# finlaymiller/torch-vae

Hardware: AMD Instinct MI355X
Metric: training samples/sec (VAE step: forward+ELBO+backward+AdamW), synthetic pianoroll (higher is better)
Workload: dtype bf16; 1 GPU; VanillaVAE latent_dim=16, 128x128 synthetic pianoroll, batch 256/GPU (generalised bottleneck 256*(H/16)^2); img_size=128, latent_dim=16, batch_per_gpu=256, global_batch=256, parallelism=dp1, optimizer=AdamW+OneCycle (encoder, decoder groups)

## Files before the change

### torch_vae_amd/csrc/vae_api.hip

```cpp
#include <map>
#include <mutex>
#include "vae_ctx.h"
#include "edge_kernels.cuh"
#include "loglik.cuh"
#include "latent_stats.cuh"
#include "grad_clip.cuh"
#include "total_corr.cuh"

static thread_local std::string g_err;
int vae_set_error(const char* what, const char* why) {
    g_err = std::string(what) + ": " + why;
    return -1;
}

extern "C" const char* vae_last_error(void) { return g_err.c_str(); }
extern "C" int vae_abi_version(void) { return 1; }

static void param_shapes(int H, int L, int gen, int64_t* sizes) {
    const int s = gen ? H / 16 : 2;
    const int64_t F = 256LL * s * s;
    const int enc_ci[4] = {1, 32, 64, 128}, enc_co[4] = {32, 64, 128, 256};
    int k = 0;
    for (int i = 0; i < 4; ++i) { sizes[k++] = 9LL * enc_ci[i] * enc_co[i]; sizes[k++] = enc_co[i]; sizes[k++] = enc_co[i]; sizes[k++] = enc_co[i]; }
    sizes[k++] = L * F; sizes[k++] = L; sizes[k++] = L * F; sizes[k++] = L; sizes[k++] = F * L; sizes[k++] = F;
    const int dec_ci[3] = {256, 128, 64}, dec_co[3] = {128, 64, 32};
    for (int i = 0; i < 3; ++i) { sizes[k++] = 9LL * dec_ci[i] * dec_co[i]; sizes[k++] = dec_co[i]; sizes[k++] = dec_co[i]; sizes[k++] = dec_co[i]; }
    sizes[k++] = 9 * 32 * 32; sizes[k++] = 32; sizes[k++] = 32; sizes[k++] = 32; sizes[k++] = 9 * 32; sizes[k++] = 1;
}

extern "C" int vae_param_layout(int H, int L, int gen, int64_t* offsets, int64_t* sizes, int64_t* total) {
    if (H < 32 || (H & (H - 1)) || (!gen && H != 32)) return vae_set_error("vae_param_layout", "img_size must be a power of two >= 32 (exactly 32 unless generalised)");
    if (L < 1 || L > 4096) return vae_set_error("vae_param_layout", "latent_dim must be in 1..4096");
    param_shapes(H, L, gen, sizes);
    int64_t off = 0;
    for (int i = 0; i < VAE_NUM_PARAMS; ++i) { offsets[i] = off; off += align_up(sizes[i], 64); }
    *total = off;
    return 0;
}
extern "C" int vae_bn_layout(int64_t* offsets, int64_t* channels, int64_t* total) {
    int64_t off = 0;
    for (int i = 0; i < 8; ++i) { offsets[i] = off; channels[i] = kBnC[i]; off += 2 * kBnC[i]; }
    *total = off;
    return 0;
}

template <typename T> static T* dalloc(vae_ctx* c, size_t n) {
    void* p = nullptr;
    if (hipMalloc(&p, std::max<size_t>(n * sizeof(T), 256)) != hipSuccess) return nullptr;
    c->allocs.push_back(p); c->ws_bytes += (int64_t)std::max<size_t>(n * sizeof(T), 256);
    return reinterpret_cast<T*>(p);
}

struct DevStreams { hipStream_t side[vae_ctx::NSIDE]; hipStream_t comm; };
static DevStreams* device_streams(int side_prio) {
    static std::mutex mu;
    static std::map<int, DevStreams*> pool;
    int dev = 0;
    if (hipGetDevice(&dev) != hipSuccess) return nullptr;
    std::lock_guard<std::mutex> lk(mu);
    auto it = pool.find(dev);
    if (it != pool.end()) return it->second;
    DevStreams* d = new DevStreams();
    bool ok = true;
    for (int i = 0; i < vae_ctx::NSIDE && ok; ++i) ok = hipStreamCreateWithPriority(&d->side[i], hipStreamNonBlocking, side_prio) == hipSuccess;
    {
        int lo = 0, hi = 0;
        (void)hipDeviceGetStreamPriorityRange(&lo, &hi);
        const char* e = getenv("VAE_COMM_STREAM_PRIO");
        if (e && (!strcmp(e, "high") || !strcmp(e, "low"))) ok = ok && hipStreamCreateWithPriority(&d->comm, hipStreamNonBlocking, !strcmp(e, "high") ? hi : lo) == hipSuccess;
        else ok = ok && hipStreamCreateWithFlags(&d->comm, hipStreamNonBlocking) == hipSuccess;
    }
    if (!ok) { delete d; return nullptr; }
    pool[dev] = d;
    return d;
}

extern "C" void vae_destroy(vae_ctx* c) {
    if (!c) return;
    (void)vae_comm_destroy(c);
    for (void* p : c->allocs) (void)hipFree(p);
    if (c->ll_kb) (void)hipFree(c->ll_kb);
    if (c->n_side_ok) {
        for (int i = 0; i < vae_ctx::NSIDE; ++i) { (void)hipStreamSynchronize(c->side[i]); (void)hipEventDestroy(c->ev_join[i]); }
        (void)hipStreamSynchronize(c->comm);
        for (int i = 0; i < vae_ctx::NFORK; ++i) (void)hipEventDestroy(c->ev_fork[i]);
        (void)hipEventDestroy(c->ev_pack); (void)hipEventDestroy(c->ev_comm);
        if (c->ev_kl) (void)hipEventDestroy(c->ev_kl);
        for (int i = 0; i < vae_ctx::NBUCKET; ++i) (void)hipEventDestroy(c->ev_bucket[i]);
    }
    delete c;
}
extern "C" int64_t vae_workspace_bytes(const vae_ctx* c) { return c ? c->ws_bytes : 0; }

struct OptionDef { const char* name; int& (*ref)(vae_ctx&); int def; int (*norm)(int); };
static int opt_any(int v) { return v; }
static int opt_min1(int v) { return std::max(1, v); }
static int opt_fused_grid(int v) { return std::max(1, std::min(v, 512)); }
static int opt_max1024(int v) { return std::min(v, 1024); }
static int opt_max48(int v) { return std::min(v, 48); }
static int opt_fused_wgrad(int v) { return v == 1 ? 3 : v == 2 ? 1 : v == 3 ? 2 : 0; }
#define OPT(member, def, norm) {#member, [](vae_ctx& c) -> int& { return c.member; }, def, norm}
#define OPT_WK(member, def, norm) {"knob_wgrad_" #member, [](vae_ctx& c) -> int& { return c.wk.member; }, def, norm}
static const OptionDef kOptions[] = {
    OPT(use_tr16, 1, opt_any), OPT(use_mfma_convout, 1, opt_any), OPT(use_pipelined, 1, opt_any), OPT(use_side_stream, 1, opt_any),
    OPT(use_fused_bn, 1, opt_any), OPT(use_fused_convout, 1, opt_any), OPT(use_fused_wgrad, 1, opt_fused_wgrad), OPT(use_recomp_dz, 0, opt_any),
    OPT(use_raw_wgrad, 0, opt_any), OPT(use_deep, 1, opt_any), OPT(use_latent_mfma, 6, opt_any), OPT(use_convout_stream, 1, opt_any),
    OPT(use_dnf_stream, 1, opt_any), OPT(use_upf_stream, 1, opt_any), OPT(use_fc_dgrad8, 1, opt_any), OPT(use_wgrad_split, 1, opt_any),
    OPT(knob_up_per_cu, 2, opt_any), OPT(knob_down_per_cu, 2, opt_min1), OPT(knob_bwd_per_cu, 0, opt_any), OPT(knob_nt_max, 4, opt_any),
    OPT(knob_up_nt_max, 1, opt_min1), OPT(knob_wave_nt_max, 4, opt_any), OPT(knob_lay22_min_nt, 2, opt_any), OPT(knob_lay42, 1, opt_any),
    OPT(knob_down_waves, 8, opt_any), OPT(knob_pipe_max_cout, 256, opt_any), OPT(knob_xcd_map, 1, opt_any), OPT(knob_rev, 4, opt_any),
    OPT(knob_lean, 1, opt_any), OPT(knob_pack_grid, 128, opt_min1), OPT(knob_conv1_grid, 512, opt_any), OPT(knob_fused_grid, 256, opt_fused_grid),
    OPT(knob_convout_grid, 1536, opt_any), OPT(knob_convout_bwd_grid, 1024, opt_any), OPT(knob_convout_step_grid, 1024, opt_min1),
    OPT(knob_convout_bands, 0, opt_any), OPT(knob_wgrad_layer_wgs, 0, opt_any), OPT(knob_skip_wgrad, 0, opt_any), OPT(knob_ablate_b, 0, opt_any),
    OPT(knob_ablate_f, 0, opt_any),
    OPT_WK(tile, 1, opt_any), OPT_WK(wide, 1, opt_any), OPT_WK(mid8, 0, opt_any), OPT_WK(force_simple, 0, opt_any),
    OPT_WK(wgs, 128, opt_max1024), OPT_WK(wide_wgs, 128, opt_max1024), OPT_WK(cap_mb, 48, opt_max48),
};
#undef OPT_WK
#undef OPT
static const OptionDef* find_option(const char* name) {
    for (const OptionDef& o : kOptions) if (name && !strcmp(name, o.name)) return &o;
    return nullptr;
}

extern "C" vae_ctx* vae_create(int H, int L, int maxB, int dtype, int gen) {
    vae_ctx* c = new vae_ctx();
    c->H = H; c->L = L; c->maxB = maxB; c->dtype = dtype; c->gen = gen;
    for (const OptionDef& o : kOptions) o.ref(*c) = o.norm(o.def);
    if (getenv("VAE_NO_SIDE_STREAM")) c->use_side_stream = 0;
    if (vae_param_layout(H, L, gen, c->poff, c->psz, &c->ptotal) != 0) { delete c; return nullptr; }
    if (dtype != VAE_DTYPE_F32 && dtype != VAE_DTYPE_BF16 && dtype != VAE_DTYPE_F16) { vae_set_error("vae_create", "bad dtype"); delete c; return nullptr; }
    if (maxB < 1) { vae_set_error("vae_create", "max_batch < 1"); delete c; return nullptr; }
    vae_bn_layout(c->bnoff, c->bnc, &c->bntotal);
    c->s = gen ? H / 16 : 2; c->s2 = c->s * c->s; c->F = 256LL * c->s2;
    c->npad_fc = (int)align_up(2 * L, 32); c->npad_di = (int)align_up(L, 32);
    c->esz = dtype == VAE_DTYPE_F32 ? 4 : 2;
    const size_t B = maxB;
    const int hs[8] = {H / 2, H / 4, H / 8, H / 16, 2 * c->s, 4 * c->s, 8 * c->s, 16 * c->s};
    size_t nd = 0;
    for (int i = 0; i < 8; ++i) nd += 4 * kBnC[i];
    nd *= STAT_R;
    c->n_dstats = nd + 8 * STAT_R;
    c->dstats = dalloc<double>(c, c->n_dstats);
    bool ok = c->dstats != nullptr;
    double* dp = c->dstats;
    for (int i = 0; i < 8 && ok; ++i) {
        BnLayer& l = c->lay[i];
        l.C = kBnC[i]; l.H = hs[i]; l.W = hs[i];
        l.stat_f = dp; dp += 2 * l.C * STAT_R;
        const size_t n = B * l.H * l.W * l.C;
        l.y = dalloc<char>(c, n * c->esz); l.dz = dalloc<char>(c, n * c->esz); l.block = dalloc<float>(c, LC_ROWS * l.C);
        ok = l.y && l.dz && l.block;
        const int base = i < 4 ? 4 * i : (i < 7 ? 22 + 4 * (i - 4) : 34);
        l.p_convw = base; l.p_convb = base + 1; l.p_gamma = base + 2; l.p_beta = base + 3;
    }
    for (int i = 0; i < 8; ++i) { c->lay[i].stat_b = dp; dp += 2 * kBnC[i] * STAT_R; }
    c->accum = dp;
    if (ok) {
        c->d0 = dalloc<char>(c, B * c->F * c->esz); c->dd0 = dalloc<char>(c, B * c->F * c->esz);
        c->eps = dalloc<float>(c, B * L); c->dlat = dalloc<float>(c, B * 2 * L);
        c->dlogit = dalloc<float>(c, B * H * H); c->dlogit2 = dalloc<float>(c, B * H * H); c->ident = dalloc<float>(c, 3 * 256); c->wout_t = dalloc<float>(c, 288);
        ok = c->d0 && c->dd0 && c->eps && c->dlat && c->dlogit && c->dlogit2 && c->ident && c->wout_t;
    }
    const int ci[8] = {1, 32, 64, 128, 256, 128, 64, 32}, co[8] = {32, 64, 128, 256, 128, 64, 32, 32};
    for (int i = 1; i < 8 && ok; ++i) {
        const size_t n = (size_t)9 * ci[i] * co[i];
        c->wp_fwd[i] = dalloc<char>(c, n * c->esz); c->wp_dg[i] = dalloc<char>(c, n * c->esz);
        ok = c->wp_fwd[i] && c->wp_dg[i];
    }
    if (ok) {
        c->fcpack = dalloc<char>(c, (size_t)c->F * c->npad_fc * c->esz);
        c->dipack = dalloc<char>(c, (size_t)c->F * c->npad_di * c->esz);
        c->d_descs = dalloc<PackDesc>(c, 32);
        ok = c->fcpack && c->dipack && c->d_descs;
    }
    size_t slab = 2048 * 288;
    if (ok) {
        int a, b2, wa, wb;
        for (int wide = 0; wide < 2; ++wide)
            for (int big = 0; big < 2; ++big) {
                if (wide && dtype == VAE_DTYPE_F32) continue;
                for (int i = 1; i < 4; ++i) slab = std::max(slab, wgrad_slab_floats(c->wk, maxB, c->lay[i].H, c->lay[i].W, co[i], ci[i], &a, &b2, &wa, &wb, wide != 0, big != 0));
                for (int i = 4; i < 8; ++i) slab = std::max(slab, wgrad_slab_floats(c->wk, maxB, c->lay[i].H / 2, c->lay[i].W / 2, ci[i], co[i], &a, &b2, &wa, &wb, wide != 0, big != 0));
            }
        const size_t ksteps = c->F / 16;
        slab = std::max(slab, (size_t)std::min<size_t>(ksteps, 512) * maxB * c->npad_fc);
        slab = std::max(slab, (size_t)std::min<size_t>(ksteps, 512) * maxB * c->npad_di);
        slab = std::max(slab, (size_t)8 * (2 * (size_t)L * c->F + c->F));
        c->slab_floats = slab;
        c->slab = dalloc<float>(c, slab);
// ... 933 lines not shown
```

### torch_vae_amd/csrc/vae_ctx.h

```cpp
#pragma once
#include <hip/hip_runtime.h>
#include <stdio.h>
#include <string.h>
#include <math.h>
#include <string>
#include <vector>
#include <algorithm>

#include "../../include/vae_step.h"

int vae_set_error(const char* what, const char* why);

#include "common.cuh"

#define LAUNCH_CHECK(name)                                                        \
    do {                                                                          \
        hipError_t _e = hipGetLastError();                                        \
        if (_e != hipSuccess) return vae_set_error(name, hipGetErrorString(_e)); \
    } while (0)

static const int kBnC[8] = {32, 64, 128, 256, 128, 64, 32, 32};
static const char* const kLayerTag[8] = {"encoder.0", "encoder.1", "encoder.2", "encoder.3", "decoder.0", "decoder.1", "decoder.2", "final_layer.0"};
static const float kSlope = 0.01f;
static const float kBnEps = 1e-5f;
static const float kBnMom = 0.1f;

static inline int64_t align_up(int64_t v, int64_t a) { return (v + a - 1) / a * a; }
static inline int ilog2(int v) { int l = 0; while ((1 << l) < v) ++l; return l; }

struct Tiling { int lth, ltw, lTB, tiles_x, tiles_y; };
static Tiling make_tiling(int Hs, int Ws, int pixels) {
    const int tw = std::min(Ws, pixels >= 128 ? 16 : 8), th = std::min(Hs, pixels / tw), TB = pixels / (th * tw);
    Tiling t; t.lth = ilog2(th); t.ltw = ilog2(tw); t.lTB = ilog2(TB); t.tiles_x = Ws / tw; t.tiles_y = Hs / th;
    return t;
}

struct BnLayer {
    int C, H, W;
    double* stat_f; double* stat_b; float* block; void* y; void* dz;
    int p_gamma, p_beta, p_convw, p_convb;
    void* act = nullptr; void* dy = nullptr; int act_ok = 0, dy_ok = 0;
};

struct PackDesc {
    const float* src; const float* src2; void* dst;
    int kind;
    int A, Bc, k_is_first, npad, L, s2;
    long n;
};

struct WgradKnobs { int wgs, cap_mb, tile, wide, wide_wgs, small_wgs = 1024, mid8, force_simple; };

struct FwdRecord {
    enum Kind { NONE, FULL, ENCODE, DECODE };
    Kind kind = NONE;
    int B = 0, trained = 0;
    int recon = VAE_RECON_BCE, kl_kind = VAE_KL_PLAIN; double kl_param = 0.0;
    int kl_pending = 0;
    int kl_reduced = 0;
    int tc_done = 0;
    const float* x = nullptr; float *xhat = nullptr, *mu = nullptr, *lv = nullptr, *z = nullptr;
    float gmul = 1.f, ginv = 1.f;
    int convout_pending = 0, dlogit_valid = 0; BnFuse pending_f7; float* loss_out3 = nullptr; float loss_kw = 0.f;
    int bwd_dirty = 1;
    int bwd_half_done = 0;
    int walk_dir = 0;
    explicit operator bool() const { return kind != NONE; }
};

struct vae_ctx {
    int H, L, maxB, dtype, gen, s, s2; int64_t F; int npad_fc, npad_di; size_t esz;
    int64_t poff[VAE_NUM_PARAMS], psz[VAE_NUM_PARAMS], ptotal, bnoff[8], bnc[8], bntotal;
    BnLayer lay[8];
    void *d0, *dd0;
    float *eps, *dlat, *dlogit, *dlogit2, *ident, *wout_t;
    void* wp_fwd[8]; void* wp_dg[8];
    void *fcpack, *dipack;
    PackDesc* d_descs; std::vector<PackDesc> h_descs; const float* packed_for = nullptr;
    float* slab; size_t slab_floats;
    static constexpr int NSIDE = 3, NFORK = 16;
    hipStream_t side[NSIDE]; float* side_slab[NSIDE]; hipEvent_t ev_fork[NFORK], ev_join[NSIDE], ev_pack; int side_rr = 0, fork_rr = 0, n_side_ok = 0;
    static constexpr int NBUCKET = 2; hipEvent_t ev_bucket[NBUCKET];
    hipStream_t comm; hipEvent_t ev_comm; int comm_busy = 0;
    void* nccl_comm = nullptr; int comm_rank = 0, comm_world = 0;
    double* dstats; size_t n_dstats; double* accum;
    float* reduce_tmp = nullptr; size_t reduce_tmp_floats = 0; unsigned reduce_slot = 0;
    float* fused_slab[3] = {nullptr, nullptr, nullptr}; size_t fused_slab_floats = 0;
    static constexpr int KL_SIDE = 2;
    void* kl_ws = nullptr; unsigned* kl_tk = nullptr; hipEvent_t ev_kl = nullptr;
    unsigned long long* kl_d() const { return static_cast<unsigned long long*>(kl_ws); }
    double* kl_scal() const { return reinterpret_cast<double*>(kl_d() + L); }
    float* kl_factor() const { return reinterpret_cast<float*>(kl_scal() + 2); }
    const double* kl_shaped() const { return fwd.kl_kind != VAE_KL_PLAIN ? kl_scal() : nullptr; }
    void* tc_ws = nullptr; size_t tc_ws_bytes = 0; int tc_ws_B = 0;
    float* tc_grad() const { return static_cast<float*>(tc_ws); }
    double* ps_part = nullptr; int ps_tb = 0, ps_ntile = 0;
    float* ll_f = nullptr; double* ll_part = nullptr; double* ll_lat = nullptr;
    double* ll_kb = nullptr; size_t ll_kb_n = 0;
    std::vector<void*> allocs; int64_t ws_bytes = 0;
    int use_tr16, use_mfma_convout, use_pipelined, use_side_stream, use_fused_bn, use_fused_convout, use_fused_wgrad, use_recomp_dz, use_raw_wgrad,
        use_deep, use_latent_mfma, use_convout_stream, use_dnf_stream, use_upf_stream, use_fc_dgrad8, use_wgrad_split;
    int knob_up_per_cu, knob_down_per_cu, knob_bwd_per_cu, knob_nt_max, knob_up_nt_max, knob_wave_nt_max, knob_lay22_min_nt, knob_lay42,
        knob_down_waves, knob_pipe_max_cout, knob_xcd_map, knob_rev, knob_lean, knob_pack_grid, knob_conv1_grid, knob_fused_grid,
        knob_convout_grid, knob_convout_bwd_grid, knob_convout_step_grid, knob_convout_bands, knob_wgrad_layer_wgs,
        knob_skip_wgrad, knob_ablate_b, knob_ablate_f;
    WgradKnobs wk;
    int recon = VAE_RECON_BCE, kl_kind = VAE_KL_PLAIN; double kl_param = 0.0;
    FwdRecord fwd;
    long long* dbg_buf = nullptr; char dbg_tag[32] = {0}; int dbg_epi = 0;
    int prof = 0; const char* tag = nullptr; struct ProfRec { std::string name; hipEvent_t e0, e1; double bytes, flops; int side; int launches = 1; }; std::vector<ProfRec> prof_recs;
    hipStream_t cur_stream = nullptr; bool cur_stream_set = false;
};

struct ProfScope {
    vae_ctx* c; hipStream_t st; int idx;
    ProfScope(vae_ctx* c_, const char* name, double bytes, double flops, hipStream_t st_) : c(c_), st(st_), idx(-1) {
        if (!c || !c->prof) return;
        vae_ctx::ProfRec r; r.name = std::string(name) + (c->tag ? std::string(" @") + c->tag : std::string()); r.bytes = bytes; r.flops = flops;
        r.side = (c->cur_stream_set && st != c->cur_stream) ? 1 : 0;
        if (hipEventCreate(&r.e0) != hipSuccess || hipEventCreate(&r.e1) != hipSuccess) return;
        (void)hipEventRecord(r.e0, st);
        c->prof_recs.push_back(r); idx = (int)c->prof_recs.size() - 1;
    }
    ~ProfScope() { if (idx >= 0) (void)hipEventRecord(c->prof_recs[idx].e1, st); }
    ProfScope(const ProfScope&) = delete;
    ProfScope& operator=(const ProfScope&) = delete;
};

static inline size_t wgrad_slab_floats(const WgradKnobs& k, int B, int Hs, int Ws, int CA, int CB, int* nsplit_out, int* tps_out, int* WA_out, int* WB_out,
                                       bool wide_ok = false, bool big = false) {
    int WA, WB;
    if (wide_ok && k.wide && CA >= 128 && k.tile == 1) { WA = 4; WB = 1; }
    else if (CA >= 64 && CB >= 64 && k.tile == 0) { WA = 2; WB = 2; } else if (CA >= 64 && k.tile <= 1) { WA = 2; WB = 1; } else { WA = 1; WB = 1; }
    Tiling t = make_tiling(Hs, Ws, WG_KP);
    const int TB = 1 << t.lTB;
    const int n_tiles = ((B + TB - 1) / TB) * t.tiles_x * t.tiles_y;
    const int chan_tiles = (CA / (32 * WA)) * (CB / (32 * WB));
    const size_t per = (size_t)9 * CA * CB;
    int nsplit = std::max(1, (!big ? k.small_wgs : (WA == 4 ? k.wide_wgs : k.wgs)) / chan_tiles);
    const size_t cap = ((size_t)k.cap_mb << 20) / 4;
    nsplit = (int)std::min<size_t>(nsplit, std::max<size_t>(1, cap / per));
    nsplit = std::min(nsplit, n_tiles);
    const int tps = (n_tiles + nsplit - 1) / nsplit;
    nsplit = (n_tiles + tps - 1) / tps;
    *nsplit_out = nsplit; *tps_out = tps; *WA_out = WA; *WB_out = WB;
    return per * nsplit;
}

static inline void set_grad_scale(vae_ctx* c, int B) {
    c->fwd.gmul = 1.f; c->fwd.ginv = 1.f;
    if (c->dtype == VAE_DTYPE_F16) {
        const int e = std::max(0, ilog2(B) + 2 * ilog2(c->H) - 4);
        c->fwd.gmul = ldexpf(1.f, e); c->fwd.ginv = ldexpf(1.f, -e);
    }
}

static inline void enter(vae_ctx* c, hipStream_t st) { c->cur_stream = st; c->cur_stream_set = true; }

static inline void drop_forward(vae_ctx* c) {
    FwdRecord& f = c->fwd;
    f.kind = FwdRecord::NONE; f.B = 0; f.trained = 0;
    f.kl_pending = 0; f.kl_reduced = 0; f.tc_done = 0; f.convout_pending = 0; f.dlogit_valid = 0; f.loss_out3 = nullptr; f.bwd_half_done = 0;
}
static inline int begin_forward(vae_ctx* c, FwdRecord::Kind kind, int B, int train, hipStream_t st) {
    enter(c, st);
    drop_forward(c);
    HIP_CHECK_RET(hipMemsetAsync(c->dstats, 0, c->n_dstats * sizeof(double), st));
    FwdRecord& f = c->fwd;
    f.kind = kind; f.B = B; f.trained = train; f.bwd_dirty = 0; f.recon = c->recon;
    const bool elbo = kind == FwdRecord::FULL;
    f.kl_kind = elbo ? c->kl_kind : VAE_KL_PLAIN; f.kl_param = elbo ? c->kl_param : 0.0;
    f.x = nullptr; f.xhat = f.mu = f.lv = f.z = nullptr;
    if (kind != FwdRecord::DECODE) f.walk_dir = 1;
    set_grad_scale(c, B);
    return 0;
}

struct SideFork { hipStream_t st; float* slab; int rc; };
SideFork fork_side(vae_ctx* c, hipStream_t st, int which = -1);
int join_sides(vae_ctx* c, hipStream_t st);
int join_comm(vae_ctx* c, hipStream_t st);
int launch_kl_shape(vae_ctx* c, hipStream_t st);
int join_kl(vae_ctx* c, hipStream_t st);
int launch_tc(vae_ctx* c, hipStream_t st);
// ... 34 lines not shown
```

### torch_vae_amd/csrc/vae_impl.cuh

```cuda
#pragma once
#include <type_traits>
#include "vae_ctx.h"
#include "conv_mfma.cuh"
#include "conv_pipe.cuh"
#include "edge_kernels.cuh"
#include "conv_fused.cuh"
#include "conv_deep.cuh"
#include "latent_mfma.cuh"
#include "convout_stream.cuh"
#include "wgrad_split.cuh"
#include "upfinal_stream.cuh"
#include "dnfirst_stream.cuh"
#include "grad_paths.cuh"

template <typename K, typename... Args>
static int launch(const char* name, K kernel, dim3 grid, dim3 block, size_t lds_bytes, hipStream_t st, const Args&... args) {
    if (lds_bytes > 160 * 1024) return vae_set_error("lds", "tile needs more than 160 KiB LDS");
    if (lds_bytes > 48 * 1024) {
        hipError_t e = hipFuncSetAttribute(reinterpret_cast<const void*>(kernel), hipFuncAttributeMaxDynamicSharedMemorySize, (int)lds_bytes);
        if (e != hipSuccess) return vae_set_error("hipFuncSetAttribute", hipGetErrorString(e));
    }
    hipLaunchKernelGGL(kernel, grid, block, lds_bytes, st, args...);
    LAUNCH_CHECK(name);
    return 0;
}

template <int... Vs, typename F>
static int pick_const(const char* what, int v, F&& f) {
    int rc = 0;
    const bool found = ((v == Vs && ((rc = f(std::integral_constant<int, Vs>{})), true)) || ...);
    return found ? rc : vae_set_error(what, "no kernel variant for this value");
}
template <typename F> static int pick_bool(bool v, F&& f) { return v ? f(std::true_type{}) : f(std::false_type{}); }
template <typename F> static int pick_recon(vae_ctx* c, F&& f) {
    return c->fwd.recon == VAE_RECON_MSE ? f(std::integral_constant<int, VAE_RECON_MSE>{}) : f(std::integral_constant<int, VAE_RECON_BCE>{});
}

static int stream_bands(int B, int rows, int max_bands, int min_rows, int rows_per_tick, int fixed_ticks) {
    const int ncu = 256;
    long best = -1; int nb = 1;
    for (int cand = 1; cand <= max_bands && rows / cand >= min_rows; cand *= 2) {
        const long rounds = ((long)B * cand + ncu - 1) / ncu, cost = rounds * (rows / cand / rows_per_tick + fixed_ticks);
        if (best < 0 || cost < best) { best = cost; nb = cand; }
    }
    return nb;
}

template <typename T> static bool fits_i32(const ConvArgs<T>& a) { return 4.0 * a.B * a.Hs * a.Ws * std::max(a.Cin, a.Cout) * sizeof(T) < 4294967296.0 && 4.0 * a.B * a.Hs * a.Ws * std::max(a.Cin, a.Cout) < 2147483648.0; }
template <typename T> static bool will_pipe(vae_ctx* c, const ConvArgs<T>& a) { return c->use_pipelined && a.Cout <= c->knob_pipe_max_cout && fits_i32(a); }
template <typename T>
static bool raw_wgrad_ok(vae_ctx* c, int i) {
    return sizeof(T) == 2 && c->use_raw_wgrad && c->use_pipelined && c->wk.wide && c->wk.tile == 1 && !c->wk.force_simple && i >= 2 && i <= 5;
}

template <typename A> static void apply_tiling(A& a, const Tiling& t) {
    a.lth = t.lth; a.ltw = t.ltw; a.lTB = t.lTB; a.tiles_x = t.tiles_x; a.tiles_y = t.tiles_y;
    a.m_tx = fastdiv_magic(t.tiles_x); a.m_txy = fastdiv_magic(t.tiles_x * t.tiles_y);
}
template <typename T> static ProfScope conv_prof(vae_ctx* c, const ConvArgs<T>& a, bool is_down, hipStream_t st) {
    const double px_lo = (double)a.B * a.Hs * a.Ws, px_hi = 4 * px_lo;
    const double px_in = is_down ? px_hi : px_lo, px_out = is_down ? px_lo : px_hi;
    return ProfScope(c, is_down ? (a.epi == EPI_FWD ? "down_fwd(conv)" : "down_bwd(convT dgrad)") : (a.epi == EPI_FWD ? "up_fwd(convT)" : "up_bwd(conv dgrad)"),
                     sizeof(T) * (px_in * a.Cin * ((a.two_src & 1) ? 2 : 1) + px_out * a.Cout * (a.epi == EPI_BWD ? 2 : 1) + 9.0 * a.Cin * a.Cout),
                     2.0 * 9 * a.Cin * a.Cout * px_lo, st);
}

template <typename T>
static int launch_conv_deep(vae_ctx* c, ConvArgs<T> a, bool is_down, hipStream_t st) {
    if constexpr (sizeof(T) != 2) return 1;
    else {
        if (!(c->use_deep & (is_down ? 1 : 2)) || !fits_i32(a) || a.stage_out || c->knob_ablate_b) return 1;
        const int NCO = is_down ? 128 : 64;
        if (a.Cout % NCO || a.Cin % 32 || a.Cin > 256) return 1;
        if (((a.two_src & 1) != 0) != (a.epi != EPI_FWD)) return 1;
        if (!is_down && a.epi == EPI_PLAIN) return 1;
        Tiling t = make_tiling(a.Hs, a.Ws, 128);
        const int TB = 1 << t.lTB, th = 1 << t.lth, tw = 1 << t.ltw;
        if (!((tw == 16 && th == 8 && TB == 1) || (tw == 8 && th == 8 && TB == 2))) return 1;
        if ((a.two_src & 1) && a.slope != 1.f) return vae_set_error("conv_deep", "gradient operands are loaded without LeakyReLU (slope must be 1)");
        apply_tiling(a, t);
        const int n_mt = ((a.B + TB - 1) / TB) * t.tiles_x * t.tiles_y, ntn = a.Cout / NCO, n_pairs = n_mt * ntn;
        a.n_mt = n_mt; a.rev = ((c->knob_rev >> 2) & 1) ? ((a.epi == EPI_FWD) ? ((c->knob_rev >> 4) & 1) : 1) : 0;
        DeepConvArgs<T> d; memset(&d, 0, sizeof(d));
        const int PH = is_down ? 2 * th + 1 : th + 1;
        if (is_down) { d.rowp = tw == 16 ? 40 : 20; d.halfw = tw + 1; }
        else { d.rowp = tw == 16 ? 32 : 24; d.halfw = 0; }
        d.imgp = PH * d.rowp; d.npl = TB * d.imgp;
        d.m_rowp = fastdiv_magic(d.rowp); d.m_imgp = fastdiv_magic(d.imgp);
        if (d.npl > 64 * (is_down ? 12 : 7)) return vae_set_error("conv_deep", "patch larger than the producers' slot table");
// ... 429 lines not shown
        else if (!(c->knob_lean & 1) && draw_eps(st)) return -1;
        LatentFwdArgs la;
        la.slab = c->slab; la.nslab = nsplit; la.npad = c->npad_fc; la.bmu = params + c->poff[17]; la.bvar = params + c->poff[19];
        la.eps = c->eps; la.mu = mu; la.lv = lv; la.z = z; la.accum = c->accum; la.B = B; la.L = L;
        return launch("latent_fwd_kernel", latent_fwd_kernel, dim3((B * L * LAT_LANES + 255) / 256), dim3(256), 0, st, la);
    }
}

template <typename T>
int forward_impl(vae_ctx* c, const float* x, int B, const float* params, float* bn_running, int64_t* nbt,
                        const float* eps, uint64_t seed, int train, float* xhat, float* mu, float* lv, float* z, hipStream_t st) {
    const int rc = encode_impl<T>(c, x, B, params, bn_running, nbt, eps, seed, train, mu, lv, z, st);
    if (rc) return rc;
    if (c->fwd.kl_kind != VAE_KL_PLAIN && launch_kl_shape(c, st)) return -1;
    if (c->fwd.kl_kind == VAE_KL_TC && launch_tc(c, st)) return -1;
    return decode_impl<T>(c, z, B, params, bn_running, nbt, train, x, xhat, st);
}


template <typename T>
static bool convt_fused_ok(vae_ctx* c, int i) {
    if (sizeof(T) != 2) return false;
    const BnLayer& l = c->lay[i]; const BnLayer& lp = c->lay[i - 1];
    const int Hs = l.H / 2, Ws = l.W / 2, CLO = lp.C;
    if (!(c->use_fused_wgrad & 1) || !c->use_pipelined || l.C != 32 || (CLO != 32 && CLO != 64) || Hs % 8 || Ws % 16) return false;
    if (4.0 * c->fwd.B * Hs * Ws * 32 * sizeof(T) >= 4294967296.0 || 1.0 * c->fwd.B * Hs * Ws * CLO * sizeof(T) >= 4294967296.0) return false;
    const int grid = std::min(c->fwd.B * (Ws / 16) * (Hs / 8), c->knob_fused_grid);
    return (size_t)grid * 9 * CLO * 32 <= c->fused_slab_floats;
}
template <typename T>
static int launch_convt_fused(vae_ctx* c, int i, const float* params, float* grads, hipStream_t st, bool recomp = false,
                              const float* dl_src = nullptr, const float* dl_scale = nullptr) {
    if constexpr (sizeof(T) != 2) return 1;
    else {
        if (!convt_fused_ok<T>(c, i)) return 1;
        const BnLayer& l = c->lay[i]; const BnLayer& lp = c->lay[i - 1];
        const int Hs = l.H / 2, Ws = l.W / 2, CLO = lp.C;
        const int fs = i == 7 ? 0 : 1;
        ConvTFusedArgs<T> a; memset(&a, 0, sizeof(a));
        a.dz = reinterpret_cast<const T*>(l.dz); a.y = reinterpret_cast<const T*>(l.y); a.gcoef = l.block + LC_P0 * l.C;
        if (bn_bwd_for(c, i, true, params, grads, &a.fuse, st)) return -1;
        a.wp = reinterpret_cast<const T*>(c->wp_dg[i]);
        a.yprev = reinterpret_cast<const T*>(lp.y); a.ocoef = lp.block; a.dzprev = reinterpret_cast<T*>(lp.dz); a.stat = lp.stat_b;
        a.slab = c->fused_slab[fs]; a.slope = kSlope;
        a.B = c->fwd.B; a.Hs = Hs; a.Ws = Ws; a.tiles_x = Ws / 16; a.tiles_y = Hs / 8; a.n_tiles = c->fwd.B * a.tiles_x * a.tiles_y;
        a.rev = (c->knob_rev >> 2) & 1;
        a.dlogit = dl_src; a.gscale = dl_scale; a.gmul = c->fwd.gmul; a.wout = c->wout_t; a.fcoef = l.block;
        if (recomp && (CLO != 32 || !dl_src)) return vae_set_error("convt_fused", "recomputed dz: final_layer.0 only");
        const int grid = std::min(a.n_tiles, c->knob_fused_grid);
        const size_t lds = convt_fused_lds(CLO, recomp);
        const double px = (double)c->fwd.B * Hs * Ws;
        {
            ProfScope ps(c, recomp ? "convT_bwd_fused(dz recomputed+dgrad+wgrad)" : "convT_bwd_fused(dgrad+wgrad)",
                         sizeof(T) * ((recomp ? 1.0 : 2.0) * 4 * px * 32 + 2.0 * px * CLO + 9.0 * 32 * CLO) + 4.0 * 9 * 32 * CLO + (recomp ? 4.0 * 4 * px : 0.0),
                         2.0 * 2 * 9 * 32 * CLO * px + (recomp ? 2.0 * 9 * 32 * 4 * px : 0.0), st);
            const auto go = [&](auto kernel) { return launch("convt_bwd_fused_kernel", kernel, dim3(grid), dim3(512), lds, st, a); };
            if (recomp ? go(convt_bwd_fused_kernel<T, 32, true>) : CLO == 32 ? go(convt_bwd_fused_kernel<T, 32>) : go(convt_bwd_fused_kernel<T, 64>)) return -1;
        }
        SideFork f = fork_side(c, st);
        if (f.rc) return -1;
        return launch_reduce(a.slab, grid, (size_t)9 * CLO * 32, grads + c->poff[l.p_convw], CLO, 32, f.st, c);
    }
}

template <typename T>
static int launch_conv_fused(vae_ctx* c, int i, const float* params, float* grads, hipStream_t st) {
    if constexpr (sizeof(T) != 2) return 1;
    else {
        const BnLayer& l = c->lay[i]; const BnLayer& lp = c->lay[i - 1];
        const int Hs = l.H, Ws = l.W;
        if (!(c->use_fused_wgrad & 2) || !c->use_pipelined || l.C != 64 || lp.C != 32 || Hs % 8 || Ws % 8) return 1;
        if (4.0 * c->fwd.B * Hs * Ws * 32 * sizeof(T) >= 4294967296.0 || 1.0 * c->fwd.B * Hs * Ws * 64 * sizeof(T) >= 4294967296.0) return 1;
        ConvFusedArgs<T> a; memset(&a, 0, sizeof(a));
        a.tiles_x = Ws / 8; a.tiles_y = Hs / 8; a.n_tiles = c->fwd.B * a.tiles_x * a.tiles_y;
        const int grid = std::min(a.n_tiles, c->knob_fused_grid);
        if ((size_t)grid * 9 * 64 * 32 > c->fused_slab_floats) return 1;
        a.dz = reinterpret_cast<const T*>(l.dz); a.y = reinterpret_cast<const T*>(l.y); a.gcoef = l.block + LC_P0 * l.C;
        if (bn_bwd_for(c, i, true, params, grads, &a.fuse, st)) return -1;
        a.wp = reinterpret_cast<const T*>(c->wp_dg[i]);
        a.yprev = reinterpret_cast<const T*>(lp.y); a.ocoef = lp.block; a.dzprev = reinterpret_cast<T*>(lp.dz); a.stat = lp.stat_b;
        a.slab = c->fused_slab[2]; a.slope = kSlope; a.B = c->fwd.B; a.Hs = Hs; a.Ws = Ws; a.rev = (c->knob_rev >> 2) & 1; a.ablate = c->knob_ablate_f;
        const double px = (double)c->fwd.B * Hs * Ws;
        {
            ProfScope ps(c, "conv_bwd_fused(dgrad+wgrad)", sizeof(T) * (2.0 * px * 64 + 2.0 * 4 * px * 32 + 9.0 * 32 * 64) + 4.0 * 9 * 32 * 64,
                         2.0 * 2 * 9 * 32 * 64 * px, st);
            if (launch("conv_bwd_fused_kernel", conv_bwd_fused_kernel<T>, dim3(grid), dim3(512), conv_fused_lds(), st, a)) return -1;
        }
        SideFork f = fork_side(c, st);
        if (f.rc) return -1;
        return launch_reduce(a.slab, grid, (size_t)9 * 64 * 32, grads + c->poff[l.p_convw], 64, 32, f.st, c);
    }
}

template <typename T>
static int wgrad_on_side(vae_ctx* c, WgradArgs<T> w, float* dw_out, hipStream_t st, bool raw = false) {
    SideFork f = fork_side(c, st);
    if (f.rc) return f.rc;
    return launch_wgrad<T>(c, w, dw_out, f.st, f.slab, raw);
}

template <typename T>
static int backward_conv_layer(vae_ctx* c, int i, const float* params, float* grads, hipStream_t st) {
    const bool convt = i >= 4, from_d0 = i == 4;
    const BnLayer& l = c->lay[i]; const BnLayer& lp = c->lay[i - 1];
    const T* dz = reinterpret_cast<const T*>(l.dz); const T* y = reinterpret_cast<const T*>(l.y); const float* gcoef = l.block + LC_P0 * l.C;
    const T* yprev = reinterpret_cast<const T*>(from_d0 ? c->d0 : lp.y); const float* cprev = from_d0 ? c->ident : lp.block;
    const float slope_prev = from_d0 ? 1.f : kSlope; const int Cprev = from_d0 ? 256 : lp.C;
    const int B = c->fwd.B, Hs = convt ? l.H / 2 : l.H, Ws = convt ? l.W / 2 : l.W;
    WgradArgs<T> w; memset(&w, 0, sizeof(w));
    if (convt) {
        w.s0 = yprev; w.scoef = cprev; w.sslope = slope_prev; w.s_two = 0; w.CA = Cprev;
        w.g0 = dz; w.g1 = y; w.gcoef = gcoef; w.gslope = 1.f; w.g_two = 1; w.CB = l.C;
    } else {
        w.s0 = dz; w.s1 = y; w.scoef = gcoef; w.sslope = 1.f; w.s_two = 1; w.CA = l.C;
        w.g0 = yprev; w.gcoef = cprev; w.gslope = slope_prev; w.g_two = 0; w.CB = Cprev;
    }
    w.B = B; w.Hs = Hs; w.Ws = Ws;
    ConvArgs<T> a; memset(&a, 0, sizeof(a));
    a.src0 = dz; a.src1 = y; a.coef = gcoef; a.slope = 1.f; a.two_src = 1;
    a.wp = reinterpret_cast<const T*>(c->wp_dg[i]);
    a.B = B; a.Hs = Hs; a.Ws = Ws; a.Cin = l.C; a.Cout = Cprev;
    if (from_d0) { a.out = reinterpret_cast<T*>(c->dd0); a.epi = EPI_PLAIN; }
    else { a.out = reinterpret_cast<T*>(lp.dz); a.yout = yprev; a.ocoef = cprev; a.oslope = kSlope; a.stat = lp.stat_b; a.epi = EPI_BWD; }
    const auto dgrad = [&] { return convt ? launch_down<T>(c, a, st) : launch_up<T>(c, a, st); };
    BnFuse fb;
    if (bn_bwd_for(c, i, will_pipe(c, a), params, grads, &fb, st)) return -1;
    w.fuse = fb; a.fuse = fb;
    const bool skip_wgrad = (c->knob_skip_wgrad >> i) & 1;
    const bool raw = raw_wgrad_ok<T>(c, i) && l.dy && will_pipe(c, a) && (from_d0 || lp.act_ok);
    if (raw) {
        a.stage_out = reinterpret_cast<T*>(l.dy);
        if (dgrad()) return -1;
        (convt ? w.g0 : w.s0) = reinterpret_cast<const T*>(l.dy); (convt ? w.s0 : w.g0) = reinterpret_cast<const T*>(from_d0 ? c->d0 : lp.act);
        w.s1 = w.g1 = nullptr; w.s_two = w.g_two = 0; w.sslope = w.gslope = 1.f; w.fuse.mode = BNF_NONE;
        return skip_wgrad ? 0 : wgrad_on_side<T>(c, w, grads + c->poff[l.p_convw], st, true);
    }
    if (!skip_wgrad && wgrad_on_side<T>(c, w, grads + c->poff[l.p_convw], st)) return -1;
    return dgrad();
}

static int bwd_clear_stats(vae_ctx* c, hipStream_t st) {
    size_t nfwd = 0;
    for (int i = 0; i < 8; ++i) nfwd += 2 * kBnC[i] * STAT_R;
    if (c->fwd.bwd_dirty) {
        HIP_CHECK_RET(hipMemsetAsync(c->dstats + nfwd, 0, nfwd * sizeof(double), st));
        for (int rep = 0; rep < STAT_R; ++rep) HIP_CHECK_RET(hipMemsetAsync(c->accum + rep * 8 + 2, 0, sizeof(double), st));
    }
    c->fwd.bwd_dirty = 1;
    return 0;
}

template <typename T>
static int backward_first(vae_ctx* c, const float* x, const float* params, float* grads, const float* g_xhat, const float* gscale,
                         const float* g_mu, const float* g_lv, const float* g_z, const float* g_pre, float kld_weight, int add_kl,
                         hipStream_t st, bool ex = false) {
    if (!c->fwd || !(c->fwd.trained || ex)) return vae_set_error("vae_backward", "no train-mode forward to differentiate");
    const int B = c->fwd.B, H = c->H, L = c->L;
    if (bwd_clear_stats(c, st)) return -1;
    const float* dl_src = c->dlogit; const float* dl_scale = gscale;
    const bool step7 = c->fwd.convout_pending != 0;
    if (step7 && (g_xhat || gscale || !add_kl)) return vae_set_error("vae_backward", "the forward ran with train = 2: only the standard ELBO backward (no upstream gradient on xhat, no loss scale) can follow");
    if (!step7 && add_kl && !c->fwd.dlogit_valid) return vae_set_error("vae_backward", "this forward's output-conv gradient was already consumed (train = 2 forwards can be differentiated once)");
    if (g_xhat || !add_kl) {
        const long n = (long)B * H * H;
        if (launch("dlogit_combine_kernel", dlogit_combine_kernel, dim3((unsigned)std::min<long>((n + 255) / 256, 4096)), dim3(256), 0, st,
                   g_xhat, c->fwd.xhat, add_kl ? c->dlogit : nullptr, gscale, c->dlogit2, n)) return -1;
        dl_src = c->dlogit2; dl_scale = nullptr;
    }
    c->tag = "final_layer.3";
// ... 278 lines not shown
```

Before: 235,000 samples/s.

## Add warp-specialized split variant of fused conv backward dgrad+wgrad kernel

Adds a 1024-thread variant of the fused conv backward kernel for the decoder layer. Eight producer waves load and BN-transform the next tile into double-buffered LDS and run the epilogue. The other waves split the MFMA work: some do dgrad by tap class, others do wgrad taps. This overlaps global loads and elementwise work with matrix math, where the old single-role 512-thread kernel did them in sequence. The new variant is enabled by default and uses more LDS and registers per workgroup, which may reduce occupancy.

```diff
diff --git a/torch_vae_amd/csrc/conv_fused_split.cuh b/torch_vae_amd/csrc/conv_fused_split.cuh
--- /dev/null
+++ b/torch_vae_amd/csrc/conv_fused_split.cuh
@@ -0,0 +1,314 @@
+#pragma once
+#include "conv_fused.cuh"
+#include "conv_deep.cuh"
+
+static inline size_t conv_fused_split_lds() {
+    return 2 * ((size_t)81 * (64 * 2 + 16) + (size_t)289 * 80) + (size_t)9 * 8 * 32 * 16 + (size_t)(3 * 64 + 64) * 4 + (size_t)256 * (32 * 4 + 16);
+}
+
+template <typename T>
+__device__ __forceinline__ void conv_fused_split_wgrad_tile(f32x16& acc, const char* gpatch, const char* apatch, int tp, int acol, int bcol, int lane) {
+    constexpr int LPW = 9, HPW = 17, LP = 64 * 2 + 16, HP = 80;
+    const int g4 = lane >> 4, q = (lane & 15) >> 2;
+    const int toff = (tp / 3) * HPW + (tp % 3);
+#pragma unroll
+    for (int ks = 0; ks < 4; ++ks) {
+        const int kk0 = ks * 16 + 8 * (g4 >> 1) + q, kk1 = kk0 + 4;
+        const int ga0 = (kk0 >> 3) * LPW + (kk0 & 7), ga1 = (kk1 >> 3) * LPW + (kk1 & 7);
+        const int gb0 = (2 * (kk0 >> 3)) * HPW + 2 * (kk0 & 7), gb1 = (2 * (kk1 >> 3)) * HPW + 2 * (kk1 & 7);
+        const Frag<T> af = frag_tr16<T>(gpatch + ga0 * LP + acol, gpatch + ga1 * LP + acol);
+        const Frag<T> bf = frag_tr16<T>(apatch + (gb0 + toff) * HP + bcol, apatch + (gb1 + toff) * HP + bcol);
+        mma(acc, af, bf);
+        if (ks & 1) __builtin_amdgcn_sched_barrier(0);
+    }
+}
+
+template <typename T, bool GRPB>
+__device__ __forceinline__ void conv_fused_split_dgrad(const char* gpatch, const char* wlds, char* ftile, int m, int r, int h) {
+    constexpr int LPW = 9, LP = 64 * 2 + 16, WT = 16, FP = 32 * 4 + 16;
+    constexpr int tap_cls[9] = {0, 1, 1, 2, 2, 3, 3, 3, 3};
+    constexpr int tap_t[9] = {4, 5, 3, 7, 1, 8, 6, 2, 0};
+    constexpr int tap_off[9] = {0, 0, 1, 0, 2, 0, 1, 2, 3};
+    const int Rr = m * 32 + r, pbase = (Rr >> 3) * LPW + (Rr & 7);
+    f32x16 dacc[GRPB ? 3 : 1];
+#pragma unroll
+    for (int cI = 0; cI < (GRPB ? 3 : 1); ++cI)
+#pragma unroll
+        for (int i = 0; i < 16; ++i) dacc[cI][i] = 0.f;
+#pragma unroll
+    for (int ks = 0; ks < 4; ++ks) {
+        Frag<T> af[4];
+#pragma unroll
+        for (int o = 0; o < 4; ++o)
+            af[o] = load_frag(reinterpret_cast<const T*>(gpatch + (pbase + (o >> 1) * LPW + (o & 1)) * LP + ks * 32) + h * 8);
+#pragma unroll
+        for (int kt = (GRPB ? 0 : 5); kt < (GRPB ? 5 : 9); ++kt) {
+            const Frag<T> bf = load_frag(reinterpret_cast<const T*>(wlds + (((tap_t[kt] * 8 + 2 * ks + h) * 32 + r) * 16)));
+            mma(dacc[GRPB ? tap_cls[kt] : 0], af[tap_off[kt]], bf);
+        }
+        __builtin_amdgcn_sched_barrier(0);
+    }
+    char* fbase = ftile + ((m * 8) * WT + 8 * h) * FP + r * 4;
+#pragma unroll
+    for (int cI = 0; cI < (GRPB ? 3 : 1); ++cI) {
+        const int cls = GRPB ? cI : 3, cpy = cls >> 1, cpx = cls & 1;
+#pragma unroll
+        for (int i = 0; i < 16; ++i)
+            *reinterpret_cast<float*>(fbase + ((2 * (i >> 2) + cpy) * WT + 2 * (i & 3) + cpx) * FP) = dacc[cI][i];
+    }
+}
+
+template <typename T>
+__global__ __launch_bounds__(1024) void conv_bwd_fused_split_kernel(ConvFusedArgs<T> a) {
+    static_assert(sizeof(T) == 2, "16-bit storage only (f32 keeps the separate kernels)");
+    typedef typename H16<T>::v8 T8;
+    constexpr int CLO = 64, TH = 8, TW = 8;
+    constexpr int LPH = TH + 1, LPW = TW + 1, NLP = LPH * LPW;
+    constexpr int HT = 2 * TH, WT = 2 * TW, NHI = HT * WT;
+    constexpr int HPH = HT + 1, HPW = WT + 1, NHP = HPH * HPW;
+    constexpr int LP = CLO * 2 + 16, HP = 80;
+    constexpr int NPT = 512;
+    constexpr int NGC = NLP * 8, NG = (NGC + NPT - 1) / NPT;
+    constexpr int NAC = NHP * 4, NA = (NAC + NPT - 1) / NPT;
+    constexpr int NWT = 4;
+    constexpr int GBUF = NLP * LP, ABUF = NHP * HP;
+    constexpr int FP = 32 * 4 + 16;
+    extern __shared__ __attribute__((aligned(16))) char smem[];
+    char* gpatch0 = smem;
+    char* apatch0 = gpatch0 + 2 * GBUF;
+    char* wlds = apatch0 + 2 * ABUF;
+    float* cfg = reinterpret_cast<float*>(wlds + 9 * 8 * 32 * 16);
+    float* cfa = cfg + 3 * CLO;
+    char* ftile = reinterpret_cast<char*>(cfa + 64);
+    const int tid = threadIdx.x, lane = tid & 63, wave = __builtin_amdgcn_readfirstlane(tid >> 6), r = lane & 31, h = lane >> 5;
+    const int Hg = 2 * a.Hs, Wg = 2 * a.Ws;
+
+    if (tid < CLO) {
+        if (a.fuse.mode == BNF_BWD) bn_fused_channel(a.fuse, tid, blockIdx.x == 0, cfg[tid], cfg[CLO + tid], cfg[2 * CLO + tid]);
+        else { cfg[tid] = a.gcoef[tid]; cfg[CLO + tid] = a.gcoef[CLO + tid]; cfg[2 * CLO + tid] = a.gcoef[2 * CLO + tid]; }
+    }
+    if (tid >= 64 && tid < 96) { const int n = tid - 64; cfa[n] = a.ocoef[LC_SC * 32 + n]; cfa[32 + n] = a.ocoef[LC_SH * 32 + n]; }
+    for (int i = tid; i < 9 * 8 * 32; i += 1024)
+        *reinterpret_cast<T8*>(wlds + i * 16) = *reinterpret_cast<const T8*>(reinterpret_cast<const char*>(a.wp) + (size_t)i * 16);
+
+    auto tile_origin = [&](int t_, int& b, int& y0, int& x0) __attribute__((always_inline)) {
+        const int t = a.rev ? a.n_tiles - 1 - t_ : t_;
+        const int tx = t % a.tiles_x, ty = (t / a.tiles_x) % a.tiles_y;
+        b = t / (a.tiles_x * a.tiles_y); y0 = ty * TH; x0 = tx * TW;
+    };
+    const int G = (int)gridDim.x, t0 = (int)blockIdx.x;
+    const int nt = t0 < a.n_tiles ? (a.n_tiles - 1 - t0) / G + 1 : 0;
+    __syncthreads();
+
+    if (wave >= 8) {
+        const int pt = tid - NPT, pwave = wave - 8;
+        int grel[NG], gmeta[NG], arel[NA], ameta[NA];
+#pragma unroll
+        for (int u = 0; u < NG; ++u) {
+            const int id = pt + NPT * u, pix = id >> 3, py = pix / LPW, px = pix - py * LPW;
+            grel[u] = (py * a.Ws + px) * CLO + (id & 7) * 8;
+            gmeta[u] = (id < NGC ? pix * LP + (id & 7) * 16 : 0xffff) | (py << 16) | (px << 24);
+        }
+#pragma unroll
+        for (int u = 0; u < NA; ++u) {
+            const int id = pt + NPT * u, pix = id >> 2, py = pix / HPW, px = pix - py * HPW;
+            arel[u] = (py * Wg + px) * 32 + (id & 3) * 8;
+            ameta[u] = (id < NAC ? pix * HP + (id & 3) * 16 : 0xffff) | (py << 16) | (px << 24);
+        }
+        T8 pz[NG], pyy[NG], pa[NA], pe[2];
+        int gok = 0, aok = 0;
+        auto issue = [&](int t) __attribute__((always_inline)) {
+            int b, y0, x0; tile_origin(t, b, y0, x0);
+            gok = 0; aok = 0;
+            const int gbase = ((b * a.Hs + y0) * a.Ws + x0) * CLO, abase = ((b * Hg + 2 * y0 - 1) * Wg + 2 * x0 - 1) * 32;
+#pragma unroll
+            for (int u = 0; u < NG; ++u) {
+                const int py = (gmeta[u] >> 16) & 0xff, px = (gmeta[u] >> 24) & 0xff;
+                const bool ok = (gmeta[u] & 0xffff) != 0xffff && y0 + py < a.Hs && x0 + px < a.Ws;
+                gok |= ok ? (1 << u) : 0;
+                const uint32_t off = ok ? (uint32_t)(gbase + grel[u]) * 2u : 0u;
+                pz[u] = *reinterpret_cast<const T8*>(at_bytes(a.dz, off));
+                pyy[u] = *reinterpret_cast<const T8*>(at_bytes(a.y, off));
+            }
+#pragma unroll
+            for (int u = 0; u < NA; ++u) {
+                const int py = (ameta[u] >> 16) & 0xff, px = (ameta[u] >> 24) & 0xff;
+                const bool ok = (ameta[u] & 0xffff) != 0xffff && (y0 > 0 || py > 0) && (x0 > 0 || px > 0);
+                aok |= ok ? (1 << u) : 0;
+                const uint32_t off = ok ? (uint32_t)(abase + arel[u]) * 2u : 0u;
+                pa[u] = *reinterpret_cast<const T8*>(at_bytes(a.yprev, off));
+            }
+        };
+        f32x2 s1[4], s2[4];
+#pragma unroll
+        for (int e = 0; e < 4; ++e) { s1[e] = f32x2{0.f, 0.f}; s2[e] = f32x2{0.f, 0.f}; }
+#pragma unroll
+        for (int u = 0; u < 2; ++u) pe[u] = T8{0, 0, 0, 0, 0, 0, 0, 0};
+        const int qq = pt & 3;
+
+        if (nt > 0) issue(t0);
+        for (int k = 0; k <= nt; ++k) {
+            const int t = t0 + k * G;
+            int eb = 0, ey0 = 0, ex0 = 0;
+            if (k >= 1) {
+                tile_origin(t - G, eb, ey0, ex0);
+                if (!VAE_ABLATE(a.ablate, 2)) {
+#pragma unroll
+                    for (int u = 0; u < 2; ++u) {
+                        const int pix = (pt + NPT * u) >> 2;
+                        const uint32_t off = (uint32_t)(((eb * Hg + 2 * ey0 + (pix >> 4)) * Wg + 2 * ex0 + (pix & 15)) * 32 + qq * 8) * 2u;
+                        pe[u] = *reinterpret_cast<const T8*>(at_bytes(a.yprev, off));
+                    }
+                }
+            }
+            if (k < nt) {
+                char* gpatch = gpatch0 + (k & 1) * GBUF;
+                char* apatch = apatch0 + (k & 1) * ABUF;
+                if (!VAE_ABLATE(a.ablate, 4)) {
+                    const int cg0 = (pt & 7) * 8;
+#pragma unroll
+                    for (int u = 0; u < NG; ++u) {
+                        const int lo_ = gmeta[u] & 0xffff;
+                        T8 o;
+#pragma unroll
+                        for (int e = 0; e < 4; ++e) {
+                            const int c = cg0 + 2 * e;
+                            const f32x2 k0 = *reinterpret_cast<const f32x2*>(cfg + c), k1 = *reinterpret_cast<const f32x2*>(cfg + CLO + c), k2 = *reinterpret_cast<const f32x2*>(cfg + 2 * CLO + c);
+                            const f32x2 x0_ = {(float)pz[u][2 * e], (float)pz[u][2 * e + 1]}, x1_ = {(float)pyy[u][2 * e], (float)pyy[u][2 * e + 1]};
+                            const f32x2 z = x0_ * k0 + (x1_ * k1 + k2);
+                            o[2 * e] = (T)z.x; o[2 * e + 1] = (T)z.y;
+                        }
+                        if (!((gok >> u) & 1)) o = T8{0, 0, 0, 0, 0, 0, 0, 0};
+                        if (lo_ != 0xffff) *reinterpret_cast<T8*>(gpatch + lo_) = o;
+                    }
+                    const int ca0 = (pt & 3) * 8;
+#pragma unroll
+                    for (int u = 0; u < NA; ++u) {
+                        const int lo_ = ameta[u] & 0xffff;
+                        T8 av;
+#pragma unroll
+                        for (int e = 0; e < 4; ++e) {
+                            const f32x2 sc2 = *reinterpret_cast<const f32x2*>(cfa + ca0 + 2 * e), sh2 = *reinterpret_cast<const f32x2*>(cfa + 32 + ca0 + 2 * e);
+                            f32x2 z = f32x2{(float)pa[u][2 * e], (float)pa[u][2 * e + 1]} * sc2 + sh2;
+                            const f32x2 zs = z * a.slope;
+                            z.x = fmaxf(z.x, zs.x); z.y = fmaxf(z.y, zs.y);
+                            av[2 * e] = (T)z.x; av[2 * e + 1] = (T)z.y;
+                        }
+                        if (!((aok >> u) & 1)) av = T8{0, 0, 0, 0, 0, 0, 0, 0};
+                        if (lo_ != 0xffff) *reinterpret_cast<T8*>(apatch + lo_) = av;
+                    }
+                }
+                if (k + 1 < nt && !VAE_ABLATE(a.ablate, 8)) issue(t + G);
+            }
+            deep::barrier_lds();
+            if (k >= 1 && !VAE_ABLATE(a.ablate, 2)) {
+                f32x2 esc2[4], esh2[4];
+#pragma unroll
+                for (int e = 0; e < 4; ++e) { esc2[e] = *reinterpret_cast<const f32x2*>(cfa + qq * 8 + 2 * e); esh2[e] = *reinterpret_cast<const f32x2*>(cfa + 32 + qq * 8 + 2 * e); }
+#pragma unroll
+                for (int u = 0; u < 2; ++u) {
+                    const int pix = (pt + NPT * u) >> 2;
+                    const T8 yv8 = pe[u];
+                    const f32x4 a0_ = *reinterpret_cast<const f32x4*>(ftile + pix * FP + qq * 32), a1_ = *reinterpret_cast<const f32x4*>(ftile + pix * FP + qq * 32 + 16);
+                    T8 o;
+#pragma unroll
+                    for (int e = 0; e < 4; ++e) {
+                        const f32x2 yv = {(float)yv8[2 * e], (float)yv8[2 * e + 1]};
+                        const f32x2 z = yv * esc2[e] + esh2[e];
+                        f32x2 g = e < 2 ? f32x2{a0_[2 * e], a0_[2 * e + 1]} : f32x2{a1_[2 * e - 4], a1_[2 * e - 3]};
+                        g.x = z.x > 0.f ? g.x : g.x * a.slope; g.y = z.y > 0.f ? g.y : g.y * a.slope;
+                        T o0, o1;
+                        const f32x2 dzv = round_pair<T>(g, o0, o1);
+                        o[2 * e] = o0; o[2 * e + 1] = o1;
+                        s1[e] += dzv; s2[e] += dzv * yv;
+                    }
+                    const uint32_t off = (uint32_t)(((eb * Hg + 2 * ey0 + (pix >> 4)) * Wg + 2 * ex0 + (pix & 15)) * 32 + qq * 8) * 2u;
+                    *reinterpret_cast<T8*>(at_bytes(a.dzprev, off)) = o;
+                }
+            }
+            deep::barrier_lds();
+        }
+        float* redw = reinterpret_cast<float*>(ftile);
+#pragma unroll
+        for (int e = 0; e < 4; ++e) {
+            float v[4] = {s1[e].x, s1[e].y, s2[e].x, s2[e].y};
+#pragma unroll
+            for (int kk = 0; kk < 4; ++kk) {
+#pragma unroll
+                for (int o = 4; o < 64; o <<= 1) v[kk] += __shfl_xor(v[kk], o, 64);
+            }
+            if (lane < 4) {
+                const int c = lane * 8 + 2 * e;
+                redw[(pwave * 32 + c) * 2] = v[0]; redw[(pwave * 32 + c + 1) * 2] = v[1];
+                redw[(pwave * 32 + c) * 2 + 1] = v[2]; redw[(pwave * 32 + c + 1) * 2 + 1] = v[3];
+            }
+        }
+    } else if (wave < 2) {
+        for (int k = 0; k <= nt; ++k) {
+            if (k >= 1 && !VAE_ABLATE(a.ablate, 1))
+                conv_fused_split_dgrad<T, true>(gpatch0 + ((k - 1) & 1) * GBUF, wlds, ftile, wave & 1, r, h);
+            deep::barrier_lds();
+            deep::barrier_lds();
+        }
+    } else if (wave < 4) {
+        const int g4 = lane >> 4, p = lane & 3;
+        const int acol = ((wave & 1) * 32 + 16 * (g4 & 1) + 4 * p) * 2, bcol = (16 * (g4 & 1) + 4 * p) * 2;
+        f32x16 wacc;
+#pragma unroll
+        for (int i = 0; i < 16; ++i) wacc[i] = 0.f;
+        const bool mm = !VAE_ABLATE(a.ablate, 1);
+        for (int k = 0; k <= nt; ++k) {
+            const char* gpatch = gpatch0 + ((k - 1) & 1) * GBUF;
+            const char* apatch = apatch0 + ((k - 1) & 1) * ABUF;
+            if (k >= 1 && mm) conv_fused_split_dgrad<T, false>(gpatch, wlds, ftile, wave & 1, r, h);
+            deep::barrier_lds();
+            if (k >= 1 && mm) conv_fused_split_wgrad_tile<T>(wacc, gpatch, apatch, 8, acol, bcol, lane);
+            deep::barrier_lds();
+        }
+#pragma unroll
+        for (int i = 0; i < 16; ++i)
+            a.slab[(((size_t)blockIdx.x * 9 + 8) * CLO + (wave & 1) * 32 + acc_row(i, lane)) * 32 + r] = wacc[i];
+    } else {
+        const int g4 = lane >> 4, li = lane & 15, p = li & 3;
+        const int wj = wave - 4;
+        const int acol = ((wj & 1) * 32 + 16 * (g4 & 1) + 4 * p) * 2, bcol = (16 * (g4 & 1) + 4 * p) * 2;
+        f32x16 wacc[NWT];
+#pragma unroll
+        for (int j = 0; j < NWT; ++j)
+#pragma unroll
+            for (int i = 0; i < 16; ++i) wacc[j][i] = 0.f;
+        const bool mm = !VAE_ABLATE(a.ablate, 1);
+        for (int k = 0; k <= nt; ++k) {
+            const char* gpatch = gpatch0 + ((k - 1) & 1) * GBUF;
+            const char* apatch = apatch0 + ((k - 1) & 1) * ABUF;
+            if (k >= 1 && mm) {
+#pragma unroll
+                for (int j = 0; j < 2; ++j) conv_fused_split_wgrad_tile<T>(wacc[j], gpatch, apatch, (wj + 4 * j) >> 1, acol, bcol, lane);
+            }
+            deep::barrier_lds();
+            if (k >= 1 && mm) {
+#pragma unroll
+                for (int j = 2; j < NWT; ++j) conv_fused_split_wgrad_tile<T>(wacc[j], gpatch, apatch, (wj + 4 * j) >> 1, acol, bcol, lane);
+            }
+            deep::barrier_lds();
+        }
+#pragma unroll
+        for (int j = 0; j < NWT; ++j) {
+            const int idx = wj + 4 * j, tp = idx >> 1, cib = idx & 1;
+#pragma unroll
+            for (int i = 0; i < 16; ++i)
+                a.slab[(((size_t)blockIdx.x * 9 + tp) * CLO + cib * 32 + acc_row(i, lane)) * 32 + r] = wacc[j][i];
+        }
+    }
+    __syncthreads();
+    if (tid < 32) {
+        const float* redw = reinterpret_cast<const float*>(ftile);
+        float v1 = 0.f, v2 = 0.f;
+#pragma unroll
+        for (int w = 0; w < 8; ++w) { v1 += redw[(w * 32 + tid) * 2]; v2 += redw[(w * 32 + tid) * 2 + 1]; }
+        v2 = a.ocoef[LC_INVSTD * 32 + tid] * v2 + a.ocoef[LC_XM * 32 + tid] * v1;
+        double* st_ = a.stat + stat_rep() * 64;
+        unsafeAtomicAdd(&st_[tid], (double)v1);
+        unsafeAtomicAdd(&st_[32 + tid], (double)v2);
+    }
+}
diff --git a/torch_vae_amd/csrc/vae_api.hip b/torch_vae_amd/csrc/vae_api.hip
--- a/torch_vae_amd/csrc/vae_api.hip
+++ b/torch_vae_amd/csrc/vae_api.hip
@@ -106,6 +106,7 @@
     OPT(use_fused_bn, 1, opt_any), OPT(use_fused_convout, 1, opt_any), OPT(use_fused_wgrad, 1, opt_fused_wgrad), OPT(use_recomp_dz, 0, opt_any),
     OPT(use_raw_wgrad, 0, opt_any), OPT(use_deep, 1, opt_any), OPT(use_latent_mfma, 6, opt_any), OPT(use_convout_stream, 1, opt_any),
     OPT(use_dnf_stream, 1, opt_any), OPT(use_upf_stream, 1, opt_any), OPT(use_fc_dgrad8, 1, opt_any), OPT(use_wgrad_split, 1, opt_any),
+    OPT(use_fused_split, 1, opt_any),
     OPT(knob_up_per_cu, 2, opt_any), OPT(knob_down_per_cu, 2, opt_min1), OPT(knob_bwd_per_cu, 0, opt_any), OPT(knob_nt_max, 4, opt_any),
     OPT(knob_up_nt_max, 1, opt_min1), OPT(knob_wave_nt_max, 4, opt_any), OPT(knob_lay22_min_nt, 2, opt_any), OPT(knob_lay42, 1, opt_any),
     OPT(knob_down_waves, 8, opt_any), OPT(knob_pipe_max_cout, 256, opt_any), OPT(knob_xcd_map, 1, opt_any), OPT(knob_rev, 4, opt_any),
diff --git a/torch_vae_amd/csrc/vae_ctx.h b/torch_vae_amd/csrc/vae_ctx.h
--- a/torch_vae_amd/csrc/vae_ctx.h
+++ b/torch_vae_amd/csrc/vae_ctx.h
@@ -99,7 +99,7 @@
     double* ll_kb = nullptr; size_t ll_kb_n = 0;
     std::vector<void*> allocs; int64_t ws_bytes = 0;
     int use_tr16, use_mfma_convout, use_pipelined, use_side_stream, use_fused_bn, use_fused_convout, use_fused_wgrad, use_recomp_dz, use_raw_wgrad,
-        use_deep, use_latent_mfma, use_convout_stream, use_dnf_stream, use_upf_stream, use_fc_dgrad8, use_wgrad_split;
+        use_deep, use_latent_mfma, use_convout_stream, use_dnf_stream, use_upf_stream, use_fc_dgrad8, use_wgrad_split, use_fused_split;
     int knob_up_per_cu, knob_down_per_cu, knob_bwd_per_cu, knob_nt_max, knob_up_nt_max, knob_wave_nt_max, knob_lay22_min_nt, knob_lay42,
         knob_down_waves, knob_pipe_max_cout, knob_xcd_map, knob_rev, knob_lean, knob_pack_grid, knob_conv1_grid, knob_fused_grid,
         knob_convout_grid, knob_convout_bwd_grid, knob_convout_step_grid, knob_convout_bands, knob_wgrad_layer_wgs,
diff --git a/torch_vae_amd/csrc/vae_impl.cuh b/torch_vae_amd/csrc/vae_impl.cuh
--- a/torch_vae_amd/csrc/vae_impl.cuh
+++ b/torch_vae_amd/csrc/vae_impl.cuh
@@ -5,6 +5,7 @@
 #include "conv_pipe.cuh"
 #include "edge_kernels.cuh"
 #include "conv_fused.cuh"
+#include "conv_fused_split.cuh"
 #include "conv_deep.cuh"
 #include "latent_mfma.cuh"
 #include "convout_stream.cuh"
@@ -600,9 +601,10 @@
         a.slab = c->fused_slab[2]; a.slope = kSlope; a.B = c->fwd.B; a.Hs = Hs; a.Ws = Ws; a.rev = (c->knob_rev >> 2) & 1; a.ablate = c->knob_ablate_f;
         const double px = (double)c->fwd.B * Hs * Ws;
         {
-            ProfScope ps(c, "conv_bwd_fused(dgrad+wgrad)", sizeof(T) * (2.0 * px * 64 + 2.0 * 4 * px * 32 + 9.0 * 32 * 64) + 4.0 * 9 * 32 * 64,
+            ProfScope ps(c, c->use_fused_split ? "conv_bwd_fused(dgrad+wgrad; split)" : "conv_bwd_fused(dgrad+wgrad)", sizeof(T) * (2.0 * px * 64 + 2.0 * 4 * px * 32 + 9.0 * 32 * 64) + 4.0 * 9 * 32 * 64,
                          2.0 * 2 * 9 * 32 * 64 * px, st);
-            if (launch("conv_bwd_fused_kernel", conv_bwd_fused_kernel<T>, dim3(grid), dim3(512), conv_fused_lds(), st, a)) return -1;
+            if (c->use_fused_split ? launch("conv_bwd_fused_split_kernel", conv_bwd_fused_split_kernel<T>, dim3(grid), dim3(1024), conv_fused_split_lds(), st, a)
+                                   : launch("conv_bwd_fused_kernel", conv_bwd_fused_kernel<T>, dim3(grid), dim3(512), conv_fused_lds(), st, a)) return -1;
         }
         SideFork f = fork_side(c, st);
         if (f.rc) return -1;
```

Result: no change. 237,100 samples/s, median of 6 (+0.9%).
